# MatthewZhang473/Efficient-Gaussian-Process-on-Graphs

Hardware: NVIDIA B200
Metric: grf_walk_steps_per_sec (higher is better)
Workload: dtype f64 walk loads / f32 matvec

## Files before the change

### efficient-gaussian-process-on-graphs_b200/csrc/grf_transpose.cu

```cuda

#include "grf_common.cuh"

namespace grf {

constexpr int kRadixThreads = 256;
constexpr int kRadixWarps = kRadixThreads / 32;
constexpr int kRadixItems = 16;
constexpr int kRadixTile = kRadixThreads * kRadixItems;
constexpr int kRadixMaxBits = 10;

__global__ void __launch_bounds__(256) transpose_keys_kernel(const int32_t *__restrict__ blk_ptr,
                                                             const int2 *__restrict__ entries, int64_t n_rows,
                                                             int32_t L, int32_t entry_lo,
                                                             uint32_t *__restrict__ keys, int2 *__restrict__ payload) {
    const int lane = threadIdx.x & 31;
    const int64_t warp0 = ((int64_t)blockIdx.x * blockDim.x + threadIdx.x) >> 5;
    const int64_t nwarps = ((int64_t)gridDim.x * blockDim.x) >> 5;
    for (int64_t r = warp0; r < n_rows; r += nwarps) {
        const int32_t b = __ldg(blk_ptr + r * L), e = __ldg(blk_ptr + (r + 1) * L);
        for (int32_t i = b + lane; i < e; i += 32) {
            const int2 en = __ldg(entries + i);
            const uint32_t col = (uint32_t)en.x & kColMask, len = (uint32_t)en.x >> kStepShift;
            keys[i - entry_lo] = col * (uint32_t)L + len;
            payload[i - entry_lo] = make_int2((int32_t)((len << kStepShift) | (uint32_t)r), en.y);
        }
    }
}

__global__ void __launch_bounds__(kRadixThreads) radix_hist_kernel(const uint32_t *__restrict__ keys, int64_t n,
                                                                   int32_t shift, int32_t nbins,
                                                                   int32_t tiles_per_cta,
                                                                   int32_t *__restrict__ hist) {
    extern __shared__ uint32_t sh_hist[];
    for (int d = threadIdx.x; d < nbins; d += kRadixThreads) sh_hist[d] = 0u;
    __syncthreads();
    const uint32_t mask = (uint32_t)nbins - 1u;
    const int64_t begin = (int64_t)blockIdx.x * tiles_per_cta * kRadixTile;
    const int64_t end = min(n, begin + (int64_t)tiles_per_cta * kRadixTile);
    for (int64_t i0 = begin + threadIdx.x; i0 < end; i0 += (int64_t)kRadixThreads * 4) {
        uint32_t k[4];
#pragma unroll
        for (int u = 0; u < 4; ++u) {
            const int64_t i = i0 + (int64_t)u * kRadixThreads;
            k[u] = i < end ? __ldg(keys + i) : 0u;
        }
#pragma unroll
        for (int u = 0; u < 4; ++u) {
            const int64_t i = i0 + (int64_t)u * kRadixThreads;
            if (i < end) atomicAdd(&sh_hist[(k[u] >> shift) & mask], 1u);
        }
    }
    __syncthreads();
    for (int d = threadIdx.x; d < nbins; d += kRadixThreads) hist[(int64_t)d * gridDim.x + blockIdx.x] = (int32_t)sh_hist[d];
}

__device__ __forceinline__ uint32_t smem_u32(const void *p) { return (uint32_t)__cvta_generic_to_shared(p); }
__device__ __forceinline__ void mbar_init(uint64_t *bar, uint32_t count) {
    asm volatile("mbarrier.init.shared::cta.b64 [%1], %0;" ::"r"(count), "r"(smem_u32(bar)));
}
__device__ __forceinline__ void mbar_expect_tx(uint64_t *bar, uint32_t bytes) {
    asm volatile("mbarrier.arrive.expect_tx.shared::cta.b64 _, [%1], %0;" ::"r"(bytes), "r"(smem_u32(bar)) : "memory");
}
__device__ __forceinline__ void mbar_wait(uint64_t *bar, uint32_t parity) {
    asm volatile(
        "{\n\t"
        ".reg .pred P1;\n\t"
        "WAIT_LOOP:\n\t"
        "mbarrier.try_wait.parity.shared::cta.b64 P1, [%0], %1;\n\t"
        "@P1 bra DONE;\n\t"
        "bra WAIT_LOOP;\n\t"
        "DONE:\n\t"
        "}" ::"r"(smem_u32(bar)),
        "r"(parity)
        : "memory");
}
__device__ __forceinline__ void bulk_g2s(void *smem_dst, const void *gmem_src, uint32_t bytes, uint64_t *bar) {
    asm volatile("cp.async.bulk.shared::cluster.global.mbarrier::complete_tx::bytes [%0], [%1], %2, [%3];" ::"r"(
                     smem_u32(smem_dst)),
                 "l"(gmem_src), "r"(bytes), "r"(smem_u32(bar))
                 : "memory");
}

template <bool kLast>
__global__ void __launch_bounds__(kRadixThreads, 2) radix_scatter_kernel(const uint32_t *__restrict__ keys_in,
                                                                         const int2 *__restrict__ pay_in,
                                                                         int64_t n, int32_t shift, int32_t nbins,
                                                                         int32_t tiles_per_cta,
                                                                         const int32_t *__restrict__ offsets,
                                                                         uint32_t *__restrict__ keys_out,
                                                                         int2 *__restrict__ pay_out) {
    extern __shared__ __align__(128) unsigned char sh_bytes[];
    int2 *spay = reinterpret_cast<int2 *>(sh_bytes);
    uint32_t *skey0 = reinterpret_cast<uint32_t *>(spay + kRadixTile);
    unsigned short *xsrc = reinterpret_cast<unsigned short *>(skey0 + 2 * kRadixTile);
    uint32_t *gbase = reinterpret_cast<uint32_t *>(xsrc + kRadixTile);
    uint32_t *dstart = gbase + nbins;
    unsigned short *cnt = reinterpret_cast<unsigned short *>(dstart + nbins);
    __shared__ uint32_t warp_sums[kRadixWarps];
    __shared__ __align__(8) uint64_t bar_key[2], bar_pay;
    const int w = threadIdx.x >> 5, lane = threadIdx.x & 31;
    const uint32_t mask = (uint32_t)nbins - 1u;
    const unsigned lt = (1u << lane) - 1u;
    const int dpt = nbins >= kRadixThreads ? nbins / kRadixThreads : 1;
    const int d0 = threadIdx.x * dpt;
    const bool owner = d0 < nbins;
    const int64_t begin = (int64_t)blockIdx.x * tiles_per_cta * kRadixTile;
    const int64_t end = min(n, begin + (int64_t)tiles_per_cta * kRadixTile);
    if (begin >= end) return;
    for (int d = threadIdx.x; d < nbins; d += kRadixThreads) gbase[d] = (uint32_t)offsets[(int64_t)d * gridDim.x + blockIdx.x];
    auto key_bytes = [&](int64_t tile) { return (uint32_t)(((min((int64_t)kRadixTile, end - tile) * 4) + 15) & ~15ll); };
    auto pay_bytes = [&](int64_t tile) { return (uint32_t)(((min((int64_t)kRadixTile, end - tile) * 8) + 15) & ~15ll); };
    if (threadIdx.x == 0) {
        mbar_init(&bar_key[0], 1);
        mbar_init(&bar_key[1], 1);
        mbar_init(&bar_pay, 1);
        asm volatile("fence.mbarrier_init.release.cluster;" ::: "memory");
        mbar_expect_tx(&bar_key[0], key_bytes(begin));
        bulk_g2s(skey0, keys_in + begin, key_bytes(begin), &bar_key[0]);
        mbar_expect_tx(&bar_pay, pay_bytes(begin));
        bulk_g2s(spay, pay_in + begin, pay_bytes(begin), &bar_pay);
        if (begin + kRadixTile < end) {
            mbar_expect_tx(&bar_key[1], key_bytes(begin + kRadixTile));
            bulk_g2s(skey0 + kRadixTile, keys_in + begin + kRadixTile, key_bytes(begin + kRadixTile), &bar_key[1]);
        }
    }
    unsigned short *mycnt = cnt + w * nbins;
    uint32_t it = 0;
    for (int64_t tile = begin; tile < end; tile += kRadixTile, ++it) {
        const uint32_t *skey = skey0 + (it & 1u) * kRadixTile;
        {
            uint32_t *z = reinterpret_cast<uint32_t *>(cnt);
            for (int i = threadIdx.x; i < nbins * kRadixWarps / 2; i += kRadixThreads) z[i] = 0u;
        }
        __syncthreads();
        mbar_wait(&bar_key[it & 1u], (it >> 1) & 1u);
        const int n_tile = (int)min((int64_t)kRadixTile, end - tile);
        unsigned short rank[kRadixItems];
        const int lbase = w * (32 * kRadixItems) + lane;
#pragma unroll
        for (int k = 0; k < kRadixItems; ++k) {
            const int li = lbase + k * 32;
            const bool valid = li < n_tile;
            const uint32_t d = valid ? (skey[li] >> shift) & mask : 0u;
            const unsigned peers = __match_any_sync(0xffffffffu, valid ? d : (0x80000000u | (uint32_t)lane));
            unsigned short prev = 0;
            if (valid) prev = mycnt[d];
            __syncwarp();
            if (valid && (peers & lt) == 0u) mycnt[d] = (unsigned short)(prev + __popc(peers));
            __syncwarp();
            rank[k] = (unsigned short)(prev + __popc(peers & lt));
        }
        __syncthreads();
        uint32_t tot[4];
        uint32_t mine = 0u;
#pragma unroll
        for (int j = 0; j < 4; ++j) {
            tot[j] = 0u;
            if (j < dpt && owner) {
                const int d = d0 + j;
                uint32_t run = 0u;
#pragma unroll
                for (int ww = 0; ww < kRadixWarps; ++ww) {
                    const uint32_t c = cnt[ww * nbins + d];
                    cnt[ww * nbins + d] = (unsigned short)run;
                    run += c;
                }
                tot[j] = run;
                mine += run;
            }
        }
        uint32_t incl = mine;
#pragma unroll
        for (int dd = 1; dd < 32; dd <<= 1) {
            const uint32_t o = __shfl_up_sync(0xffffffffu, incl, dd);
            if (lane >= dd) incl += o;
        }
        if (lane == 31) warp_sums[w] = incl;
        __syncthreads();
        uint32_t before = 0u;
#pragma unroll
        for (int ww = 0; ww < kRadixWarps; ++ww) before += ww < w ? warp_sums[ww] : 0u;
        uint32_t run = before + incl - mine;
#pragma unroll
        for (int j = 0; j < 4; ++j) {
            if (j < dpt && owner) {
                dstart[d0 + j] = run;
                run += tot[j];
            }
        }
        __syncthreads();
#pragma unroll
        for (int k = 0; k < kRadixItems; ++k) {
            const int li = lbase + k * 32;
            if (li < n_tile) {
                const uint32_t d = (skey[li] >> shift) & mask;
                xsrc[dstart[d] + mycnt[d] + rank[k]] = (unsigned short)li;
            }
        }
        __syncthreads();
        mbar_wait(&bar_pay, it & 1u);
#pragma unroll 4
        for (int i = threadIdx.x; i < n_tile; i += kRadixThreads) {
            const int src = xsrc[i];
            const uint32_t kk = skey[src];
            const uint32_t d = (kk >> shift) & mask;
            const uint32_t pos = gbase[d] + ((uint32_t)i - dstart[d]);
            if (!kLast) keys_out[pos] = kk;
            pay_out[pos] = spay[src];
        }
        __syncthreads();
#pragma unroll
        for (int j = 0; j < 4; ++j)
            if (j < dpt && owner) gbase[d0 + j] += tot[j];
        if (threadIdx.x == 0) {
            const int64_t next = tile + kRadixTile, next2 = tile + 2 * (int64_t)kRadixTile;
            if (next < end) {
                mbar_expect_tx(&bar_pay, pay_bytes(next));
                bulk_g2s(spay, pay_in + next, pay_bytes(next), &bar_pay);
            }
            if (next2 < end) {
                mbar_expect_tx(&bar_key[it & 1u], key_bytes(next2));
                bulk_g2s(skey0 + (it & 1u) * kRadixTile, keys_in + next2, key_bytes(next2), &bar_key[it & 1u]);
            }
        }
    }
}

struct RadixPlan {
    int passes;
    int bits[4];
    int grid;
    int tiles_per_cta;
};

static RadixPlan radix_plan(int64_t n_keys_space, int64_t n) {
    RadixPlan p;
    const int key_bits = bit_width((uint64_t)(n_keys_space > 1 ? n_keys_space - 1 : 1));
    p.passes = (key_bits + kRadixMaxBits - 1) / kRadixMaxBits;
    if (p.passes < 1) p.passes = 1;
    const int base = key_bits / p.passes, extra = key_bits % p.passes;
    for (int i = 0; i < p.passes; ++i) p.bits[i] = base + (i >= p.passes - extra ? 1 : 0);
    for (int i = 0; i < p.passes; ++i)
        if (p.bits[i] < 1) p.bits[i] = 1;
    const int64_t tiles = (n + kRadixTile - 1) / kRadixTile;
    int64_t grid = (int64_t)kSmCount * 2;
    if (grid > tiles) grid = tiles;
    if (grid < 1) grid = 1;
    p.grid = (int)grid;
    p.tiles_per_cta = (int)((tiles + grid - 1) / grid);
    return p;
}

static inline int64_t align16(int64_t x) { return (x + 15) / 16 * 16; }

}

using namespace grf;

static int64_t transpose_counts_bytes(int64_t n_cols, int32_t n_steps) {
    return align16((n_cols * n_steps + 2) * (int64_t)sizeof(int32_t));
}

extern "C" int64_t grf_transpose_workspace_bytes(int64_t n_cols, int32_t n_steps, int64_t nnz) {
    const RadixPlan rp = radix_plan(n_cols * n_steps, nnz);
    const int64_t hist_items = (int64_t)(1 << kRadixMaxBits) * rp.grid;
    int64_t b = transpose_counts_bytes(n_cols, n_steps) + align16(grf_scan_workspace_bytes(n_cols * n_steps)) + 32;
    b += 2 * align16(nnz * 4);
    b += (rp.passes >= 2 ? 2 : 1) * align16(nnz * 8);
    b += 2 * align16((hist_items + 1) * 4) + align16(grf_scan_workspace_bytes(hist_items));
    return b;
}

namespace grf {
__global__ void __launch_bounds__(256) transpose_count_kernel(const int32_t *blk_ptr, const GrfEntry *entries,
                                                              int64_t n_rows, int32_t L, int32_t *tcnt) {
    const int lane = threadIdx.x & 31;
    const int64_t warp0 = ((int64_t)blockIdx.x * blockDim.x + threadIdx.x) >> 5;
    const int64_t nwarps = ((int64_t)gridDim.x * blockDim.x) >> 5;
    for (int64_t r = warp0; r < n_rows; r += nwarps) {
        const int32_t b = blk_ptr[r * L], e = blk_ptr[(r + 1) * L];
        for (int32_t i = b + lane; i < e; i += 32) {
            const int32_t packed = entries[i].col;
            atomicAdd(&tcnt[(int64_t)entry_col(packed) * L + entry_step(packed)], 1);
        }
    }
}
}

static inline int grid_rows(int64_t n_rows) {
    int64_t g = (n_rows + 7) / 8;
    const int64_t cap = (int64_t)kSmCount * 32;
    if (g > cap) g = cap;
    if (g < 1) g = 1;
    return (int)g;
}

extern "C" int grf_transpose_offsets(const int32_t *blk_ptr, const GrfEntry *entries, int64_t n_rows, int64_t n_cols,
                                     int32_t n_steps, const int32_t *col_counts, int32_t *tblk_ptr, void *workspace,
                                     int32_t census_threshold, int32_t *census_host, void *stream) {
    GRF_ON_STREAM_DEVICE(stream, tblk_ptr);
    GRF_REQUIRE(n_rows >= 0 && n_cols >= 0 && n_steps >= 1, "grf_transpose_offsets: bad shape");
    GRF_REQUIRE(tblk_ptr && workspace, "grf_transpose_offsets: null buffer");
    GRF_REQUIRE(!census_host || census_threshold >= 1, "grf_transpose_offsets: bad census threshold");
    cudaStream_t st = (cudaStream_t)stream;
    int32_t *tcnt = (int32_t *)workspace;
    char *scan_ws = (char *)workspace + transpose_counts_bytes(n_cols, n_steps);
    int32_t *census = (int32_t *)(scan_ws + align16(grf_scan_workspace_bytes(n_cols * n_steps)));
    if (col_counts) {
        tcnt = const_cast<int32_t *>(col_counts);
    } else if (n_cols > 0) {
        GRF_CUDA_OK(cudaMemsetAsync(tcnt, 0, (size_t)n_cols * n_steps * sizeof(int32_t), st));
        if (n_rows > 0) {
            GRF_REQUIRE(blk_ptr, "grf_transpose_offsets: null blk_ptr");
            transpose_count_kernel<<<grid_rows(n_rows), 256, 0, st>>>(blk_ptr, entries, n_rows, n_steps, tcnt);
            GRF_CUDA_OK(cudaGetLastError());
        }
    }
    int rc = grf_scan_counts(tcnt, n_cols, n_steps, GRF_ORDER_ROW_MAJOR, tblk_ptr, 0, scan_ws, stream);
    if (rc != GRF_OK) return rc;
    if (census_host) {
        rc = grf_row_census(blk_ptr, n_rows, n_steps, census_threshold, census, stream);
        if (rc != GRF_OK) return rc;
        rc = grf_row_census(tblk_ptr, n_cols, n_steps, census_threshold, census + 3, stream);
        if (rc != GRF_OK) return rc;
        GRF_CUDA_OK(cudaMemcpyAsync(census_host, census, 6 * sizeof(int32_t), cudaMemcpyDeviceToHost, st));
    }
    return GRF_OK;
}

extern "C" int grf_transpose_fill(const int32_t *blk_ptr, const GrfEntry *entries, int64_t n_rows, int64_t n_cols,
                                  int32_t n_steps, int64_t entry_lo, int64_t nnz, void *workspace,
                                  GrfEntry *tentries, void *stream) {
    GRF_ON_STREAM_DEVICE(stream, workspace);
    GRF_REQUIRE(n_rows >= 0 && n_cols >= 0 && n_steps >= 1 && nnz >= 0 && entry_lo >= 0,
                "grf_transpose_fill: bad shape");
    GRF_REQUIRE(entry_lo + nnz < (1ll << 31), "grf_transpose_fill: entry range exceeds the 32-bit offsets");
    GRF_REQUIRE(n_cols * n_steps < (1ll << 32), "grf_transpose_fill: (column, length) keys exceed 32 bits");
    if (n_cols == 0 || n_rows == 0 || nnz == 0) return GRF_OK;
    GRF_REQUIRE(blk_ptr && entries && workspace && tentries, "grf_transpose_fill: null buffer");
    cudaStream_t st = (cudaStream_t)stream;
    const RadixPlan rp = radix_plan(n_cols * n_steps, nnz);
    char *p = (char *)workspace + transpose_counts_bytes(n_cols, n_steps) +
              align16(grf_scan_workspace_bytes(n_cols * n_steps)) + 32;
    uint32_t *keys[2];
    keys[0] = (uint32_t *)p;
    p += align16(nnz * 4);
    keys[1] = (uint32_t *)p;
    p += align16(nnz * 4);
    int2 *pay[2];
    pay[0] = (int2 *)p;
    p += align16(nnz * 8);
    pay[1] = pay[0];
    if (rp.passes >= 2) {
        pay[1] = (int2 *)p;
        p += align16(nnz * 8);
    }
    const int64_t hist_cap = (int64_t)(1 << kRadixMaxBits) * rp.grid;
    int32_t *hist = (int32_t *)p;
    p += align16((hist_cap + 1) * 4);
    int32_t *offs = (int32_t *)p;
    p += align16((hist_cap + 1) * 4);
    void *scan_ws = p;

    {
        const int max_smem = kRadixTile * (8 + 2 * 4 + 2) + (1 << kRadixMaxBits) * (8 + 2 * kRadixWarps);
        GRF_CUDA_OK(cudaFuncSetAttribute(radix_scatter_kernel<true>, cudaFuncAttributeMaxDynamicSharedMemorySize, max_smem));
        GRF_CUDA_OK(cudaFuncSetAttribute(radix_scatter_kernel<false>, cudaFuncAttributeMaxDynamicSharedMemorySize, max_smem));
    }
    transpose_keys_kernel<<<grid_rows(n_rows), 256, 0, st>>>(blk_ptr, (const int2 *)entries, n_rows, n_steps,
                                                             (int32_t)entry_lo, keys[0], pay[0]);
    GRF_CUDA_OK(cudaGetLastError());
    int shift = 0;
    int cur = 0;
    for (int pass = 0; pass < rp.passes; ++pass) {
        const int nbins = 1 << rp.bits[pass];
        const bool last = pass + 1 == rp.passes;
        radix_hist_kernel<<<rp.grid, kRadixThreads, nbins * sizeof(uint32_t), st>>>(keys[cur], nnz, shift, nbins,
                                                                                     rp.tiles_per_cta, hist);
        GRF_CUDA_OK(cudaGetLastError());
        const int rc = grf_scan_counts(hist, (int64_t)nbins * rp.grid, 1, GRF_ORDER_ROW_MAJOR, offs, 0, scan_ws, stream);
        if (rc != GRF_OK) return rc;
        const size_t smem = (size_t)kRadixTile * (8 + 2 * 4 + 2) + (size_t)nbins * 2 * sizeof(uint32_t) +
                            (size_t)nbins * kRadixWarps * sizeof(unsigned short);
        if (last) {
            radix_scatter_kernel<true><<<rp.grid, kRadixThreads, smem, st>>>(
                keys[cur], pay[cur], nnz, shift, nbins, rp.tiles_per_cta, offs, nullptr, (int2 *)tentries);
        } else {
            radix_scatter_kernel<false><<<rp.grid, kRadixThreads, smem, st>>>(
                keys[cur], pay[cur], nnz, shift, nbins, rp.tiles_per_cta, offs, keys[cur ^ 1], pay[cur ^ 1]);
        }
        GRF_CUDA_OK(cudaGetLastError());
        shift += rp.bits[pass];
        cur ^= 1;
    }
    return GRF_OK;
}
```

Measured before the change: 24.42 billion.

## Fuse key construction into first radix pass and privatize histogram counters

Drops the separate pass that materialized keys and payloads. It now writes only row indices and derives keys directly from the entries in the first histogram and scatter passes, with the payload assembled on the fly. It also widens the histogram kernel to 512 threads with 8 shared sub-histograms and vectorized uint4 key loads, which cuts atomic contention. The aim is less global memory traffic in the transpose, at the cost of extra template variants, alignment handling of the entries buffer, and a new alignment requirement.

```diff
diff --git a/efficient-gaussian-process-on-graphs_b200/csrc/grf_transpose.cu b/efficient-gaussian-process-on-graphs_b200/csrc/grf_transpose.cu
--- a/efficient-gaussian-process-on-graphs_b200/csrc/grf_transpose.cu
+++ b/efficient-gaussian-process-on-graphs_b200/csrc/grf_transpose.cu
@@ -1,5 +1,12 @@
 
 #include "grf_common.cuh"
+
+#ifdef GRF_DEBUG_BOUNDS
+#include <cassert>
+#define GRF_BOUND(i, n) assert((int64_t)(i) >= 0 && (int64_t)(i) < (int64_t)(n))
+#else
+#define GRF_BOUND(i, n) ((void)0)
+#endif
 
 namespace grf {
 
@@ -8,50 +15,91 @@
 constexpr int kRadixItems = 16;
 constexpr int kRadixTile = kRadixThreads * kRadixItems;
 constexpr int kRadixMaxBits = 10;
-
-__global__ void __launch_bounds__(256) transpose_keys_kernel(const int32_t *__restrict__ blk_ptr,
-                                                             const int2 *__restrict__ entries, int64_t n_rows,
-                                                             int32_t L, int32_t entry_lo,
-                                                             uint32_t *__restrict__ keys, int2 *__restrict__ payload) {
+constexpr int kBuildThreads = 512;
+constexpr int kSubHists = 8;
+
+__device__ __forceinline__ void hist_clear(uint32_t *sh, int nbins) {
+    for (int d = threadIdx.x; d < kSubHists * nbins; d += blockDim.x) sh[d] = 0u;
+    __syncthreads();
+}
+
+__device__ __forceinline__ void hist_flush(const uint32_t *sh, int nbins, int32_t *__restrict__ hist) {
+    __syncthreads();
+    for (int d = threadIdx.x; d < nbins; d += blockDim.x) {
+        uint32_t s = 0u;
+#pragma unroll
+        for (int h = 0; h < kSubHists; ++h) s += sh[h * nbins + d];
+        GRF_BOUND((int64_t)d * gridDim.x + blockIdx.x, (int64_t)nbins * gridDim.x);
+        hist[(int64_t)d * gridDim.x + blockIdx.x] = (int32_t)s;
+    }
+}
+
+__global__ void __launch_bounds__(256) transpose_rows_kernel(const int32_t *__restrict__ blk_ptr, int64_t n_rows,
+                                                             int32_t L, int32_t entry_lo, int32_t *__restrict__ rows) {
     const int lane = threadIdx.x & 31;
     const int64_t warp0 = ((int64_t)blockIdx.x * blockDim.x + threadIdx.x) >> 5;
     const int64_t nwarps = ((int64_t)gridDim.x * blockDim.x) >> 5;
     for (int64_t r = warp0; r < n_rows; r += nwarps) {
         const int32_t b = __ldg(blk_ptr + r * L), e = __ldg(blk_ptr + (r + 1) * L);
-        for (int32_t i = b + lane; i < e; i += 32) {
-            const int2 en = __ldg(entries + i);
-            const uint32_t col = (uint32_t)en.x & kColMask, len = (uint32_t)en.x >> kStepShift;
-            keys[i - entry_lo] = col * (uint32_t)L + len;
-            payload[i - entry_lo] = make_int2((int32_t)((len << kStepShift) | (uint32_t)r), en.y);
-        }
-    }
-}
-
-__global__ void __launch_bounds__(kRadixThreads) radix_hist_kernel(const uint32_t *__restrict__ keys, int64_t n,
+        for (int32_t i = b + lane; i < e; i += 32) rows[i - entry_lo] = (int32_t)r;
+    }
+}
+
+__device__ __forceinline__ uint32_t entry_key(int2 en, int32_t L) {
+    return ((uint32_t)en.x & kColMask) * (uint32_t)L + ((uint32_t)en.x >> kStepShift);
+}
+
+constexpr int kHistUnroll = 4;
+template <bool kEntries>
+__global__ void __launch_bounds__(kBuildThreads) radix_hist_kernel(const void *__restrict__ src, int64_t n,
                                                                    int32_t shift, int32_t nbins,
-                                                                   int32_t tiles_per_cta,
+                                                                   int32_t tiles_per_cta, int32_t L,
                                                                    int32_t *__restrict__ hist) {
     extern __shared__ uint32_t sh_hist[];
-    for (int d = threadIdx.x; d < nbins; d += kRadixThreads) sh_hist[d] = 0u;
-    __syncthreads();
+    hist_clear(sh_hist, nbins);
+    uint32_t *my = sh_hist + ((threadIdx.x >> 5) & (kSubHists - 1)) * nbins;
     const uint32_t mask = (uint32_t)nbins - 1u;
     const int64_t begin = (int64_t)blockIdx.x * tiles_per_cta * kRadixTile;
     const int64_t end = min(n, begin + (int64_t)tiles_per_cta * kRadixTile);
-    for (int64_t i0 = begin + threadIdx.x; i0 < end; i0 += (int64_t)kRadixThreads * 4) {
-        uint32_t k[4];
-#pragma unroll
-        for (int u = 0; u < 4; ++u) {
-            const int64_t i = i0 + (int64_t)u * kRadixThreads;
-            k[u] = i < end ? __ldg(keys + i) : 0u;
-        }
-#pragma unroll
-        for (int u = 0; u < 4; ++u) {
-            const int64_t i = i0 + (int64_t)u * kRadixThreads;
-            if (i < end) atomicAdd(&sh_hist[(k[u] >> shift) & mask], 1u);
-        }
-    }
-    __syncthreads();
-    for (int d = threadIdx.x; d < nbins; d += kRadixThreads) hist[(int64_t)d * gridDim.x + blockIdx.x] = (int32_t)sh_hist[d];
+    if (kEntries) {
+        const int2 *ent = reinterpret_cast<const int2 *>(src);
+        constexpr int kU = 2 * kHistUnroll;
+        for (int64_t j0 = begin + threadIdx.x; j0 < end; j0 += (int64_t)kBuildThreads * kU) {
+            int2 e[kU];
+#pragma unroll
+            for (int u = 0; u < kU; ++u) {
+                const int64_t j = j0 + (int64_t)u * kBuildThreads;
+                e[u] = j < end ? __ldg(ent + j) : make_int2(0, 0);
+            }
+#pragma unroll
+            for (int u = 0; u < kU; ++u)
+                if (j0 + (int64_t)u * kBuildThreads < end) atomicAdd(&my[(entry_key(e[u], L) >> shift) & mask], 1u);
+        }
+    } else {
+        const uint32_t *keys = reinterpret_cast<const uint32_t *>(src);
+        const int64_t nvec = end > begin ? (end - begin) >> 2 : 0;
+        const uint4 *kv = reinterpret_cast<const uint4 *>(keys + begin);
+        for (int64_t v0 = threadIdx.x; v0 < nvec; v0 += (int64_t)kBuildThreads * kHistUnroll) {
+            uint4 q[kHistUnroll];
+#pragma unroll
+            for (int u = 0; u < kHistUnroll; ++u) {
+                const int64_t v = v0 + (int64_t)u * kBuildThreads;
+                q[u] = v < nvec ? __ldg(kv + v) : make_uint4(0u, 0u, 0u, 0u);
+            }
+#pragma unroll
+            for (int u = 0; u < kHistUnroll; ++u) {
+                if (v0 + (int64_t)u * kBuildThreads < nvec) {
+                    atomicAdd(&my[(q[u].x >> shift) & mask], 1u);
+                    atomicAdd(&my[(q[u].y >> shift) & mask], 1u);
+                    atomicAdd(&my[(q[u].z >> shift) & mask], 1u);
+                    atomicAdd(&my[(q[u].w >> shift) & mask], 1u);
+                }
+            }
+        }
+        for (int64_t i = begin + nvec * 4 + threadIdx.x; i < end; i += kBuildThreads)
+            atomicAdd(&my[(__ldg(keys + i) >> shift) & mask], 1u);
+    }
+    hist_flush(sh_hist, nbins, hist);
 }
 
 __device__ __forceinline__ uint32_t smem_u32(const void *p) { return (uint32_t)__cvta_generic_to_shared(p); }
@@ -81,18 +129,29 @@
                  : "memory");
 }
 
-template <bool kLast>
+template <bool kFirst>
+struct ScatterStage {
+    static constexpr int kDigBytes = kFirst ? 8 : 4;
+    static constexpr int kPayBytes = kFirst ? 4 : 8;
+    static constexpr int kDigBuf = kRadixTile * kDigBytes + (kFirst ? 16 : 0);
+    static constexpr int kBytes = kRadixTile * kPayBytes + 2 * kDigBuf + kRadixTile * 2;
+};
+
+template <bool kFirst, bool kLast>
 __global__ void __launch_bounds__(kRadixThreads, 2) radix_scatter_kernel(const uint32_t *__restrict__ keys_in,
                                                                          const int2 *__restrict__ pay_in,
-                                                                         int64_t n, int32_t shift, int32_t nbins,
-                                                                         int32_t tiles_per_cta,
+                                                                         const int2 *__restrict__ ent_in,
+                                                                         const int32_t *__restrict__ rows_in,
+                                                                         int32_t L, int64_t n, int32_t shift,
+                                                                         int32_t nbins, int32_t tiles_per_cta,
                                                                          const int32_t *__restrict__ offsets,
                                                                          uint32_t *__restrict__ keys_out,
                                                                          int2 *__restrict__ pay_out) {
+    using Stage = ScatterStage<kFirst>;
     extern __shared__ __align__(128) unsigned char sh_bytes[];
-    int2 *spay = reinterpret_cast<int2 *>(sh_bytes);
-    uint32_t *skey0 = reinterpret_cast<uint32_t *>(spay + kRadixTile);
-    unsigned short *xsrc = reinterpret_cast<unsigned short *>(skey0 + 2 * kRadixTile);
+    unsigned char *spay = sh_bytes;
+    unsigned char *sdig0 = sh_bytes + kRadixTile * Stage::kPayBytes;
+    unsigned short *xsrc = reinterpret_cast<unsigned short *>(sdig0 + 2 * Stage::kDigBuf);
     uint32_t *gbase = reinterpret_cast<uint32_t *>(xsrc + kRadixTile);
     uint32_t *dstart = gbase + nbins;
     unsigned short *cnt = reinterpret_cast<unsigned short *>(dstart + nbins);
@@ -107,41 +166,62 @@
     const int64_t begin = (int64_t)blockIdx.x * tiles_per_cta * kRadixTile;
     const int64_t end = min(n, begin + (int64_t)tiles_per_cta * kRadixTile);
     if (begin >= end) return;
+    const int off = kFirst ? (int)(((uintptr_t)ent_in >> 3) & 1u) : 0;
     for (int d = threadIdx.x; d < nbins; d += kRadixThreads) gbase[d] = (uint32_t)offsets[(int64_t)d * gridDim.x + blockIdx.x];
-    auto key_bytes = [&](int64_t tile) { return (uint32_t)(((min((int64_t)kRadixTile, end - tile) * 4) + 15) & ~15ll); };
-    auto pay_bytes = [&](int64_t tile) { return (uint32_t)(((min((int64_t)kRadixTile, end - tile) * 8) + 15) & ~15ll); };
+    auto tile_items = [&](int64_t tile) { return min((int64_t)kRadixTile, end - tile); };
+    auto issue_dig = [&](int64_t tile, uint32_t b) {
+        uint32_t bytes;
+        const void *src;
+        if (kFirst) {
+            bytes = (uint32_t)(((off + tile_items(tile)) & ~1ll) * 8);
+            src = ent_in + tile - off;
+        } else {
+            bytes = (uint32_t)((tile_items(tile) * 4 + 15) & ~15ll);
+            src = keys_in + tile;
+        }
+        mbar_expect_tx(&bar_key[b], bytes);
+        if (bytes) bulk_g2s(sdig0 + b * Stage::kDigBuf, src, bytes, &bar_key[b]);
+    };
+    auto issue_pay = [&](int64_t tile) {
+        const uint32_t bytes = (uint32_t)((tile_items(tile) * Stage::kPayBytes + 15) & ~15ll);
+        mbar_expect_tx(&bar_pay, bytes);
+        bulk_g2s(spay, kFirst ? (const void *)(rows_in + tile) : (const void *)(pay_in + tile), bytes, &bar_pay);
+    };
+    auto key_at = [&](const unsigned char *sd, int li) -> uint32_t {
+        if (kFirst) return entry_key(reinterpret_cast<const int2 *>(sd)[off + li], L);
+        return reinterpret_cast<const uint32_t *>(sd)[li];
+    };
     if (threadIdx.x == 0) {
         mbar_init(&bar_key[0], 1);
         mbar_init(&bar_key[1], 1);
         mbar_init(&bar_pay, 1);
         asm volatile("fence.mbarrier_init.release.cluster;" ::: "memory");
-        mbar_expect_tx(&bar_key[0], key_bytes(begin));
-        bulk_g2s(skey0, keys_in + begin, key_bytes(begin), &bar_key[0]);
-        mbar_expect_tx(&bar_pay, pay_bytes(begin));
-        bulk_g2s(spay, pay_in + begin, pay_bytes(begin), &bar_pay);
-        if (begin + kRadixTile < end) {
-            mbar_expect_tx(&bar_key[1], key_bytes(begin + kRadixTile));
-            bulk_g2s(skey0 + kRadixTile, keys_in + begin + kRadixTile, key_bytes(begin + kRadixTile), &bar_key[1]);
-        }
+        issue_dig(begin, 0);
+        issue_pay(begin);
+        if (begin + kRadixTile < end) issue_dig(begin + kRadixTile, 1);
     }
     unsigned short *mycnt = cnt + w * nbins;
     uint32_t it = 0;
     for (int64_t tile = begin; tile < end; tile += kRadixTile, ++it) {
-        const uint32_t *skey = skey0 + (it & 1u) * kRadixTile;
+        const unsigned char *sdig = sdig0 + (it & 1u) * Stage::kDigBuf;
+        const int n_tile = (int)tile_items(tile);
+        if (kFirst && threadIdx.x == 0 && ((off + n_tile) & 1)) {
+            GRF_BOUND(off + n_tile - 1, kRadixTile + 2);
+            reinterpret_cast<int2 *>(sdig0 + (it & 1u) * Stage::kDigBuf)[off + n_tile - 1] = __ldg(ent_in + tile + n_tile - 1);
+        }
         {
             uint32_t *z = reinterpret_cast<uint32_t *>(cnt);
             for (int i = threadIdx.x; i < nbins * kRadixWarps / 2; i += kRadixThreads) z[i] = 0u;
         }
         __syncthreads();
         mbar_wait(&bar_key[it & 1u], (it >> 1) & 1u);
-        const int n_tile = (int)min((int64_t)kRadixTile, end - tile);
         unsigned short rank[kRadixItems];
         const int lbase = w * (32 * kRadixItems) + lane;
 #pragma unroll
         for (int k = 0; k < kRadixItems; ++k) {
             const int li = lbase + k * 32;
             const bool valid = li < n_tile;
-            const uint32_t d = valid ? (skey[li] >> shift) & mask : 0u;
+            const uint32_t d = valid ? (key_at(sdig, li) >> shift) & mask : 0u;
             const unsigned peers = __match_any_sync(0xffffffffu, valid ? d : (0x80000000u | (uint32_t)lane));
             unsigned short prev = 0;
             if (valid) prev = mycnt[d];
@@ -193,7 +273,8 @@
         for (int k = 0; k < kRadixItems; ++k) {
             const int li = lbase + k * 32;
             if (li < n_tile) {
-                const uint32_t d = (skey[li] >> shift) & mask;
+                const uint32_t d = (key_at(sdig, li) >> shift) & mask;
+                GRF_BOUND(dstart[d] + mycnt[d] + rank[k], n_tile);
                 xsrc[dstart[d] + mycnt[d] + rank[k]] = (unsigned short)li;
             }
         }
@@ -202,26 +283,33 @@
 #pragma unroll 4
         for (int i = threadIdx.x; i < n_tile; i += kRadixThreads) {
             const int src = xsrc[i];
-            const uint32_t kk = skey[src];
+            uint32_t kk;
+            int2 pay;
+            if (kFirst) {
+                const int2 en = reinterpret_cast<const int2 *>(sdig)[off + src];
+                const uint32_t len = (uint32_t)en.x >> kStepShift;
+                kk = ((uint32_t)en.x & kColMask) * (uint32_t)L + len;
+                pay = make_int2((int32_t)((len << kStepShift) | (uint32_t)reinterpret_cast<const int32_t *>(spay)[src]),
+                                en.y);
+            } else {
+                kk = reinterpret_cast<const uint32_t *>(sdig)[src];
+                pay = reinterpret_cast<const int2 *>(spay)[src];
+            }
             const uint32_t d = (kk >> shift) & mask;
             const uint32_t pos = gbase[d] + ((uint32_t)i - dstart[d]);
+            GRF_BOUND(pos, n);
             if (!kLast) keys_out[pos] = kk;
-            pay_out[pos] = spay[src];
+            pay_out[pos] = pay;
         }
         __syncthreads();
 #pragma unroll
         for (int j = 0; j < 4; ++j)
             if (j < dpt && owner) gbase[d0 + j] += tot[j];
         if (threadIdx.x == 0) {
+            asm volatile("fence.proxy.async.shared::cta;" ::: "memory");
             const int64_t next = tile + kRadixTile, next2 = tile + 2 * (int64_t)kRadixTile;
-            if (next < end) {
-                mbar_expect_tx(&bar_pay, pay_bytes(next));
-                bulk_g2s(spay, pay_in + next, pay_bytes(next), &bar_pay);
-            }
-            if (next2 < end) {
-                mbar_expect_tx(&bar_key[it & 1u], key_bytes(next2));
-                bulk_g2s(skey0 + (it & 1u) * kRadixTile, keys_in + next2, key_bytes(next2), &bar_key[it & 1u]);
-            }
+            if (next < end) issue_pay(next);
+            if (next2 < end) issue_dig(next2, it & 1u);
         }
     }
 }
@@ -338,6 +426,8 @@
     GRF_REQUIRE(n_cols * n_steps < (1ll << 32), "grf_transpose_fill: (column, length) keys exceed 32 bits");
     if (n_cols == 0 || n_rows == 0 || nnz == 0) return GRF_OK;
     GRF_REQUIRE(blk_ptr && entries && workspace && tentries, "grf_transpose_fill: null buffer");
+    GRF_REQUIRE(((uintptr_t)entries & 15) == 0 && ((uintptr_t)workspace & 15) == 0,
+                "grf_transpose_fill: entries and workspace must be 16-byte aligned");
     cudaStream_t st = (cudaStream_t)stream;
     const RadixPlan rp = radix_plan(n_cols * n_steps, nnz);
     char *p = (char *)workspace + transpose_counts_bytes(n_cols, n_steps) +
@@ -362,33 +452,42 @@
     p += align16((hist_cap + 1) * 4);
     void *scan_ws = p;
 
-    {
-        const int max_smem = kRadixTile * (8 + 2 * 4 + 2) + (1 << kRadixMaxBits) * (8 + 2 * kRadixWarps);
-        GRF_CUDA_OK(cudaFuncSetAttribute(radix_scatter_kernel<true>, cudaFuncAttributeMaxDynamicSharedMemorySize, max_smem));
-        GRF_CUDA_OK(cudaFuncSetAttribute(radix_scatter_kernel<false>, cudaFuncAttributeMaxDynamicSharedMemorySize, max_smem));
-    }
-    transpose_keys_kernel<<<grid_rows(n_rows), 256, 0, st>>>(blk_ptr, (const int2 *)entries, n_rows, n_steps,
-                                                             (int32_t)entry_lo, keys[0], pay[0]);
+    const size_t bins_smem_max = (size_t)(1 << kRadixMaxBits) * (2 * sizeof(uint32_t) + kRadixWarps * sizeof(unsigned short));
+    GRF_CUDA_OK(cudaFuncSetAttribute(radix_scatter_kernel<true, true>, cudaFuncAttributeMaxDynamicSharedMemorySize,
+                                     (int)(ScatterStage<true>::kBytes + bins_smem_max)));
+    GRF_CUDA_OK(cudaFuncSetAttribute(radix_scatter_kernel<true, false>, cudaFuncAttributeMaxDynamicSharedMemorySize,
+                                     (int)(ScatterStage<true>::kBytes + bins_smem_max)));
+    GRF_CUDA_OK(cudaFuncSetAttribute(radix_scatter_kernel<false, true>, cudaFuncAttributeMaxDynamicSharedMemorySize,
+                                     (int)(ScatterStage<false>::kBytes + bins_smem_max)));
+    GRF_CUDA_OK(cudaFuncSetAttribute(radix_scatter_kernel<false, false>, cudaFuncAttributeMaxDynamicSharedMemorySize,
+                                     (int)(ScatterStage<false>::kBytes + bins_smem_max)));
+    const int2 *ent = (const int2 *)entries + entry_lo;
+    int32_t *rows = (int32_t *)keys[0];
+    transpose_rows_kernel<<<grid_rows(n_rows), 256, 0, st>>>(blk_ptr, n_rows, n_steps, (int32_t)entry_lo, rows);
     GRF_CUDA_OK(cudaGetLastError());
     int shift = 0;
     int cur = 0;
     for (int pass = 0; pass < rp.passes; ++pass) {
         const int nbins = 1 << rp.bits[pass];
-        const bool last = pass + 1 == rp.passes;
-        radix_hist_kernel<<<rp.grid, kRadixThreads, nbins * sizeof(uint32_t), st>>>(keys[cur], nnz, shift, nbins,
-                                                                                     rp.tiles_per_cta, hist);
+        const bool first = pass == 0, last = pass + 1 == rp.passes;
+        const size_t hsmem = (size_t)kSubHists * nbins * sizeof(uint32_t);
+        if (first)
+            radix_hist_kernel<true><<<rp.grid, kBuildThreads, hsmem, st>>>(ent, nnz, shift, nbins, rp.tiles_per_cta,
+                                                                          n_steps, hist);
+        else
+            radix_hist_kernel<false><<<rp.grid, kBuildThreads, hsmem, st>>>(keys[cur], nnz, shift, nbins,
+                                                                           rp.tiles_per_cta, n_steps, hist);
         GRF_CUDA_OK(cudaGetLastError());
         const int rc = grf_scan_counts(hist, (int64_t)nbins * rp.grid, 1, GRF_ORDER_ROW_MAJOR, offs, 0, scan_ws, stream);
         if (rc != GRF_OK) return rc;
-        const size_t smem = (size_t)kRadixTile * (8 + 2 * 4 + 2) + (size_t)nbins * 2 * sizeof(uint32_t) +
-                            (size_t)nbins * kRadixWarps * sizeof(unsigned short);
-        if (last) {
-            radix_scatter_kernel<true><<<rp.grid, kRadixThreads, smem, st>>>(
-                keys[cur], pay[cur], nnz, shift, nbins, rp.tiles_per_cta, offs, nullptr, (int2 *)tentries);
-        } else {
-            radix_scatter_kernel<false><<<rp.grid, kRadixThreads, smem, st>>>(
-                keys[cur], pay[cur], nnz, shift, nbins, rp.tiles_per_cta, offs, keys[cur ^ 1], pay[cur ^ 1]);
-        }
+        const size_t bins_smem = (size_t)nbins * (2 * sizeof(uint32_t) + kRadixWarps * sizeof(unsigned short));
+        const size_t smem = (first ? ScatterStage<true>::kBytes : ScatterStage<false>::kBytes) + bins_smem;
+        uint32_t *kout = last ? nullptr : keys[cur ^ 1];
+        int2 *pout = last ? (int2 *)tentries : pay[cur ^ 1];
+        auto kern = first ? (last ? radix_scatter_kernel<true, true> : radix_scatter_kernel<true, false>)
+                          : (last ? radix_scatter_kernel<false, true> : radix_scatter_kernel<false, false>);
+        kern<<<rp.grid, kRadixThreads, smem, st>>>(keys[cur], pay[cur], ent, rows, n_steps, nnz, shift, nbins,
+                                                   rp.tiles_per_cta, offs, kout, pout);
         GRF_CUDA_OK(cudaGetLastError());
         shift += rp.bits[pass];
         cur ^= 1;
diff --git a/profiles/prof_transpose.py b/profiles/prof_transpose.py
--- /dev/null
+++ b/profiles/prof_transpose.py
@@ -0,0 +1,77 @@
+import argparse
+import ctypes
+import hashlib
+import json
+import os
+import subprocess
+import sys
+
+ROOT = os.path.dirname(os.path.dirname(os.path.abspath(__file__)))
+sys.path[:0] = [ROOT, os.path.join(ROOT, "efficient-gaussian-process-on-graphs_b200")]
+import torch
+from grf_b200 import _lib, engine, synth
+
+ap = argparse.ArgumentParser()
+ap.add_argument("--reps", type=int, default=10)
+ap.add_argument("--scale", type=int, default=22)
+ap.add_argument("--edges", type=float, default=70e6)
+ap.add_argument("--out", default=None, help="also write the JSON line here")
+args = ap.parse_args()
+dev = torch.device("cuda", 0)
+torch.cuda.set_device(dev)
+L = _lib.lib()
+
+g, _ = synth.rmat_walk_graph(args.scale, int(args.edges), seed=0, device=dev)
+phi = engine.build_phi_blocks(g, engine.WalkConfig(100, 0.1, 5, seed=42), transpose=False)
+n_rows, n_cols, n_steps, nnz = phi.n_rows, phi.n_cols, phi.n_steps, phi.nnz
+vp = ctypes.c_void_p
+st = vp(torch.cuda.current_stream().cuda_stream)
+ws = torch.empty(L.grf_transpose_workspace_bytes(n_cols, n_steps, nnz), dtype=torch.uint8, device=dev)
+tblk_ptr = torch.empty(n_cols * n_steps + 1, dtype=torch.int32, device=dev)
+tentries = torch.empty((nnz, 2), dtype=torch.int32, device=dev)
+blk, ent = vp(phi.blk_ptr.data_ptr()), vp(phi.entries.data_ptr())
+_lib.check(L.grf_transpose_offsets(blk, ent, n_rows, n_cols, n_steps, None, vp(tblk_ptr.data_ptr()),
+                                   vp(ws.data_ptr()), 256, None, st))
+
+
+def fill():
+    _lib.check(L.grf_transpose_fill(blk, ent, n_rows, n_cols, n_steps, 0, nnz, vp(ws.data_ptr()),
+                                    vp(tentries.data_ptr()), st))
+
+
+fill()
+fill()
+a, b = torch.cuda.Event(enable_timing=True), torch.cuda.Event(enable_timing=True)
+torch.cuda.synchronize()
+a.record()
+for _ in range(args.reps):
+    fill()
+b.record()
+torch.cuda.synchronize()
+ms = a.elapsed_time(b) / args.reps
+
+with torch.profiler.profile(activities=[torch.profiler.ProfilerActivity.CUDA]) as prof:
+    fill()
+    torch.cuda.synchronize()
+kernels = {}
+for e in prof.events():
+    if e.device_type == torch.autograd.DeviceType.CUDA:
+        k = kernels.setdefault(e.name, {"ms": 0.0, "launches": 0})
+        k["ms"] += e.device_time / 1e3
+        k["launches"] += 1
+for k in kernels.values():
+    k["ms"] = round(k["ms"], 4)
+
+gpu = subprocess.run(["nvidia-smi", "-i", "0", "--query-gpu=name,power.limit", "--format=csv,noheader"],
+                     capture_output=True, text=True).stdout.strip()
+line = {
+    "gpu": gpu, "library": _lib.SO_PATH, "n_rows": n_rows, "n_cols": n_cols, "L": n_steps, "nnz": nnz,
+    "fill_ms": round(ms, 3), "reps": args.reps,
+    "kernels": dict(sorted(kernels.items(), key=lambda kv: -kv[1]["ms"])),
+    "sha256_tblk_ptr": hashlib.sha256(tblk_ptr.cpu().numpy().tobytes()).hexdigest(),
+    "sha256_tentries": hashlib.sha256(tentries.cpu().numpy().tobytes()).hexdigest(),
+}
+print(json.dumps(line), flush=True)
+if args.out:
+    with open(args.out, "w") as f:
+        f.write(json.dumps(line, indent=1) + "\n")
```

Result: faster. 26.20 billion, median of 6 (+7.3%).
